# NVlabs/CenterPose

Measured on NVIDIA H100. Metric: images/sec at 512x512 DLA-34 (dla_34 + DCNv2, 7 heads, decode + PnP), higher is better.
Workload: dtype tf32x3

## Files before the change

centerpose_b200/csrc/conv_tma.cu:

```cuda
#include <cuda.h>

#include "common.cuh"
#include "umma_common.cuh"

namespace cp {
namespace {

constexpr int TM_BM = 128;
constexpr int TM_THREADS = 384;
constexpr int TM_THREADS_X3 = 512;

struct TmaConvParams {
  CUtensorMap amap[4];
  int nsrc;
  int srcC[4];
  int B, H, W, Cin, Cout, CoutPad, BN;
  int k;
  int tile_m;
  int Wt, boxh;
  int tiles_per_image;
  long long total_tiles;
  long long m_tiles;
  uint32_t slab_bytes, slab_stride;
  int SA, SB;
  const float* bias;
  const float* residual;
  int resStride, relu, res_after_relu;
  float* out;
  int outStride, out_nchw;
  int round_tf32;
  int cslab;
  int x3;
  int group;
  const unsigned char* wtiles;
  int ksplit, sps;
  float* part;
  int fuse, tph;
  const float* fuse_w[16];
  const float* fuse_b[16];
  float* fuse_out[16];
  int fuse_cout[16];
  int ipm;
  long long wstride, tstride, tiles_per_model;
};

using namespace umma;

struct TmaCtl {
  unsigned long long a_full[4], a_empty[4], a_split[4];
  unsigned long long b_full[8], b_empty[8];
};
static_assert(sizeof(TmaCtl) <= 512, "control block");

struct TileGeo {
  int n_tile, img, g0, r_lo, model;
  long long pos0;
};
template <bool MULTI>
__device__ __forceinline__ TileGeo decode_tile(const TmaConvParams& p, long long ct, int n_tiles) {
  TileGeo g;
  g.n_tile = (int)(ct % n_tiles);
  const long long m_tile = ct / n_tiles;
  g.img = 0;
  g.g0 = 0;
  g.r_lo = 0;
  g.pos0 = 0;
  g.model = 0;
  if (p.k == 3) {
    g.img = (int)(m_tile / p.tiles_per_image);
    g.g0 = (int)(m_tile - (long long)g.img * p.tiles_per_image) * p.tile_m;
    const int t = g.g0 - 1;
    g.r_lo = (t >= 0) ? t / p.Wt : -((-t + p.Wt - 1) / p.Wt);
    if (MULTI) g.model = g.img / p.ipm;
  } else if (MULTI) {
    g.model = (int)(m_tile / p.tiles_per_model);
    g.pos0 = (long long)g.model * p.ipm * p.H * p.W + (m_tile - g.model * p.tiles_per_model) * p.tile_m;
  } else {
    g.pos0 = m_tile * p.tile_m;
  }
  return g;
}

template <bool MULTI>
__device__ __forceinline__ bool tile_position(const TmaConvParams& p, const TileGeo& g, int i, int* n, int* oy, int* ox, int* m) {
  bool valid;
  if (p.k == 3) {
    const int gg = g.g0 + i;
    *oy = gg / p.Wt;
    const int xp = gg - *oy * p.Wt;
    *ox = xp - 1;
    *n = g.img;
    valid = (*oy < p.H) && (xp >= 1) && (xp <= p.W);
  } else {
    const long long pix = g.pos0 + i;
    valid = pix < (MULTI ? (long long)(g.model + 1) * p.ipm : (long long)p.B) * p.H * p.W;
    const long long pp = valid ? pix : 0;
    *ox = (int)(pp % p.W);
    const long long t = pp / p.W;
    *oy = (int)(t % p.H);
    *n = (int)(t / p.H);
  }
  *m = (int)(((size_t)*n * p.H + *oy) * p.W + *ox);
  return valid;
}

template <bool X3, bool FUSE, int BN, bool MULTI>
__global__ void __launch_bounds__(X3 ? TM_THREADS_X3 : TM_THREADS, 1) conv_tma_kernel(const __grid_constant__ TmaConvParams p) {
  extern __shared__ __align__(1024) unsigned char smem[];
  TmaCtl* ctl = reinterpret_cast<TmaCtl*>(smem);
  if (threadIdx.x == 0) griddep_launch_dependents();
  const uint32_t slabs0 = (smem_u32(smem) + 512u + 1023u) & ~1023u;
  const uint32_t rowb = (uint32_t)p.cslab * 4u;
  const uint32_t btile_bytes = (uint32_t)BN * rowb * (X3 ? 2u : 1u);
  const uint32_t a_stage = p.slab_stride * (X3 ? 2u : 1u);
  const uint32_t btiles0 = slabs0 + (uint32_t)p.SA * a_stage;
  const uint32_t drain0 = btiles0 + (uint32_t)p.SB * btile_bytes;

  const int tid = threadIdx.x, warp = tid >> 5, lane = tid & 31;
  const int n_tiles = p.CoutPad / BN;
  const int taps = p.k * p.k;
  const int KS_SPLIT = p.ksplit;
  const int sps = p.sps;
  const int KB = sps * taps;
  const int KB_all = (p.Cin / p.cslab) * taps;
  const long long total_tiles = p.total_tiles;
  const long long tph = FUSE ? p.tph : 1;
  auto tile_at = [&](long long it) { return ((long long)blockIdx.x + (it / tph) * gridDim.x) * tph + (it % tph); };

  if (tid == 0) {
    for (int s = 0; s < p.SA; ++s) {
      mbar_init(smem_u32(&ctl->a_full[s]), 1);
      mbar_init(smem_u32(&ctl->a_empty[s]), 2);
      mbar_init(smem_u32(&ctl->a_split[s]), 128);
    }
    for (int s = 0; s < p.SB; ++s) {
      mbar_init(smem_u32(&ctl->b_full[s]), 1);
      mbar_init(smem_u32(&ctl->b_empty[s]), 2);
    }
    fence_mbar_init();
  }
  __syncthreads();
  if (warp != 1) griddep_wait();

  if (warp < 4) {
    if (X3) asm volatile("setmaxnreg.dec.sync.aligned.u32 40;");
    if (warp == 0) {
      if (lane == 0) {
        int stage = 0;
        uint32_t phase = 0;
        for (long long it = 0, tile = tile_at(0); tile < total_tiles; tile = tile_at(++it)) {
          const TileGeo g = decode_tile<MULTI>(p, tile / KS_SPLIT, n_tiles);
          const int s_begin = (int)(tile % KS_SPLIT) * sps;
          for (int s = s_begin; s < s_begin + sps; ++s) {
            int src = 0, cb = 0;
            while (src + 1 < p.nsrc && s * p.cslab >= cb + p.srcC[src]) {
              cb += p.srcC[src];
              ++src;
            }
            mbar_wait(smem_u32(&ctl->a_empty[stage]), phase ^ 1u);
            const uint32_t bar = smem_u32(&ctl->a_full[stage]);
            mbar_arrive_expect_tx(bar, p.slab_bytes);
            const uint32_t dst = slabs0 + (uint32_t)stage * a_stage;
            if (p.k == 3)
              tma_load_4d(dst, &p.amap[src], s * p.cslab - cb, -1, g.r_lo - 1, g.img, bar);
            else
              tma_load_2d(dst, &p.amap[src], s * p.cslab - cb, (int)g.pos0, bar);
            if (++stage == p.SA) {
              stage = 0;
              phase ^= 1u;
            }
          }
        }
      }
      __syncwarp();
    } else if (warp == 1) {
      if (lane == 0) {
        int stage = 0;
        uint32_t phase = 0;
        for (long long it = 0, tile = tile_at(0); tile < total_tiles; tile = tile_at(++it)) {
          const unsigned char* wsrc;
          if constexpr (MULTI) {
            const TileGeo g = decode_tile<MULTI>(p, tile / KS_SPLIT, n_tiles);
            wsrc = p.wtiles + (size_t)g.model * p.tstride +
                   ((size_t)g.n_tile * KB_all + (size_t)(tile % KS_SPLIT) * KB) * btile_bytes;
          } else {
            const int n_tile = (int)((tile / KS_SPLIT) % n_tiles);
            wsrc = p.wtiles + ((size_t)n_tile * KB_all + (size_t)(tile % KS_SPLIT) * KB) * btile_bytes;
          }
          for (int kb = 0; kb < KB; ++kb) {
            mbar_wait(smem_u32(&ctl->b_empty[stage]), phase ^ 1u);
            const uint32_t bar = smem_u32(&ctl->b_full[stage]);
            mbar_arrive_expect_tx(bar, btile_bytes);
            bulk_g2s(btiles0 + (uint32_t)stage * btile_bytes, wsrc + (size_t)kb * btile_bytes, btile_bytes, bar);
            if (++stage == p.SB) {
              stage = 0;
              phase ^= 1u;
            }
          }
        }
      }
      __syncwarp();
    }
  } else if (X3 && warp >= 12) {
    asm volatile("setmaxnreg.dec.sync.aligned.u32 48;");
    const int st = tid - 384;
    int stage = 0;
    uint32_t phase = 0;
    const uint32_t nchunk = p.slab_bytes >> 4;
    for (long long it = 0, tile = tile_at(0); tile < total_tiles; tile = tile_at(++it)) {
      for (int s = 0; s < sps; ++s) {
        mbar_wait(smem_u32(&ctl->a_full[stage]), phase);
        const uint32_t hi = slabs0 + (uint32_t)stage * a_stage;
        const uint32_t lo = hi + p.slab_stride;
        for (uint32_t c0 = st; c0 < nchunk; c0 += 128 * 4) {
          float4 v[4];
#pragma unroll
          for (int u = 0; u < 4; ++u)
            if (c0 + u * 128 < nchunk) v[u] = ld_shared_v4f(hi + ((c0 + u * 128) << 4));
#pragma unroll
          for (int u = 0; u < 4; ++u) {
            if (c0 + u * 128 < nchunk) {
              float4 h, l;
              h.x = tf32_round(v[u].x); l.x = tf32_round(v[u].x - h.x);
              h.y = tf32_round(v[u].y); l.y = tf32_round(v[u].y - h.y);
              h.z = tf32_round(v[u].z); l.z = tf32_round(v[u].z - h.z);
              h.w = tf32_round(v[u].w); l.w = tf32_round(v[u].w - h.w);
              st_shared_v4f(hi + ((c0 + u * 128) << 4), h.x, h.y, h.z, h.w);
              st_shared_v4f(lo + ((c0 + u * 128) << 4), l.x, l.y, l.z, l.w);
            }
          }
        }
        fence_proxy_async_smem();
        mbar_arrive(smem_u32(&ctl->a_split[stage]));
        if (++stage == p.SA) {
          stage = 0;
          phase ^= 1u;
        }
      }
    }
  } else {
    if (X3) asm volatile("setmaxnreg.inc.sync.aligned.u32 208;");
    const int c = (warp - 4) >> 2, wt = tid & 127;
    float* dstage = reinterpret_cast<float*>(smem + (drain0 - smem_u32(smem))) + (size_t)c * (DRAIN_STAGE_BYTES / 4);
    const uint32_t bar_a = smem_u32(X3 ? &ctl->a_split[0] : &ctl->a_full[0]);
    const uint32_t bar_a_empty = smem_u32(&ctl->a_empty[0]);
    const uint32_t bar_b_full = smem_u32(&ctl->b_full[0]), bar_b_empty = smem_u32(&ctl->b_empty[0]);
    const uint32_t a_lo_u = p.slab_stride >> 4, b_lo_u = ((uint32_t)BN * rowb) >> 4;
    EpiParams ep;
    ep.bias = p.bias;
    ep.residual = p.residual;
    ep.resStride = p.resStride;
    ep.relu = p.relu;
    ep.res_after_relu = p.res_after_relu;
    ep.round_tf32 = p.round_tf32;
    ep.out = p.out;
    ep.outStride = p.outStride;
    ep.out_nchw = p.out_nchw;
    ep.Cout = p.Cout;
    ep.CoutPad = p.CoutPad;
    ep.H = p.H;
    ep.W = p.W;
    int sa = 0, sb = 0;
    uint32_t pa = 0, pb = 0;
    float acc[BN / 2];
    float sums[X3 ? BN / 2 : 1];
    float acc2[FUSE ? 16 : 1];
#pragma unroll
    for (int j = 0; j < BN / 2; ++j) acc[j] = 0.f;
#pragma unroll
    for (int j = 0; j < (FUSE ? 16 : 1); ++j) acc2[j] = 0.f;
    for (long long it = 0, tile = tile_at(0); tile < total_tiles; tile = tile_at(++it)) {
      const TileGeo g = decode_tile<MULTI>(p, tile / KS_SPLIT, n_tiles);
      const uint32_t row0 = (p.k == 3 ? (uint32_t)(g.g0 - 1 - g.r_lo * p.Wt) : 0u) + (uint32_t)c * 64u;
#pragma unroll
      for (int j = 0; j < (X3 ? BN / 2 : 1); ++j) sums[j] = 0.f;
      const int group = X3 ? p.group : 1;
      const bool overlap = X3 && p.SA > 1;
      int tap = 0;
      auto release_prev = [&]() {
        if (wt == 0) {
          mbar_arrive(bar_b_empty + 8u * (uint32_t)(sb == 0 ? p.SB - 1 : sb - 1));
          if (tap == 0) mbar_arrive(bar_a_empty + 8u * (uint32_t)(sa == 0 ? p.SA - 1 : sa - 1));
        }
      };
      for (int kb0 = 0; kb0 < KB; kb0 += group) {
        const int n_kb = min(group, KB - kb0);
        for (int i = 0; i < n_kb; ++i) {
          if (tap == 0) mbar_wait(bar_a + 8u * (uint32_t)sa, pa);
          const int ky = tap / 3, kx = tap - ky * 3;
          const uint32_t arow = row0 + (p.k == 3 ? (uint32_t)(ky * p.Wt + kx) : 0u);
          mbar_wait(bar_b_full + 8u * (uint32_t)sb, pb);
          const uint64_t da = make_desc(slabs0 + (uint32_t)sa * a_stage + arow * rowb, p.cslab);
          const uint64_t db = make_desc(btiles0 + (uint32_t)sb * btile_bytes, p.cslab);
          const bool fresh = X3 ? i == 0 : kb0 == 0;
          if (p.cslab == 32)
            mma_kblock_issue<BN, X3, false, 4>(acc, da, db, a_lo_u, b_lo_u, fresh);
          else
            mma_kblock_issue<BN, X3, false, 2>(acc, da, db, a_lo_u, b_lo_u, fresh);
          if (overlap && i > 0) {
            wg_wait<1>();
            release_prev();
          }
          if (++sb == p.SB) {
            sb = 0;
            pb ^= 1u;
          }
          if (++tap == taps) {
            tap = 0;
            if (++sa == p.SA) {
              sa = 0;
              pa ^= 1u;
            }
          }
          if (!overlap) {
            wg_wait<0>();
            release_prev();
          }
        }
        wg_wait<0>();
        if (overlap) release_prev();
#pragma unroll
        for (int j = 0; j < (X3 ? BN / 2 : 1); ++j)
          if (X3) sums[j] += acc[X3 ? j : 0];
      }
      if (X3) {
#pragma unroll
        for (int j = 0; j < BN / 2; ++j) acc[j] = 0.f;
      }
      const int r_me = wt >> 1;
      int n, oy, ox, m;
      const bool valid = tile_position<MULTI>(p, g, c * 64 + r_me, &n, &oy, &ox, &m);
      const int col_end = min(p.Cout, (g.n_tile + 1) * BN);
      const int head = FUSE ? g.n_tile / p.tph : 0, part = FUSE ? g.n_tile - head * p.tph : 0;
      const size_t wofs = MULTI ? (size_t)g.model * p.wstride : 0;
      if (MULTI) ep.bias = p.bias + wofs;
      if (FUSE && part == 0) {
#pragma unroll
        for (int j = 0; j < (FUSE ? 16 : 1); ++j) acc2[j] = 0.f;
      }
      auto fn = [&](int r, int cb, float (&v)[16]) {
        if (cb >= BN) return;
        if (!FUSE && KS_SPLIT > 1) {
          const long long mn = tile / KS_SPLIT;
          const int ks = (int)(tile % KS_SPLIT);
          float4* mine = reinterpret_cast<float4*>(p.part) + (((size_t)mn * KS_SPLIT + ks) * (BN >> 2) + (cb >> 2)) * p.tile_m +
                         c * 64 + r;
#pragma unroll
          for (int q = 0; q < 4; ++q) __stcg(mine + (size_t)q * p.tile_m, make_float4(v[4 * q], v[4 * q + 1], v[4 * q + 2], v[4 * q + 3]));
        } else if (FUSE) {
          const float* b1 = p.bias + wofs + (size_t)g.n_tile * BN + cb;
          const float4* w2 = reinterpret_cast<const float4*>(p.fuse_w[head] + wofs) + ((size_t)part * BN + cb) * 4;
#pragma unroll
          for (int q = 0; q < 16; ++q) {
            const float h = fmaxf(v[q] + __ldg(b1 + q), 0.f);
#pragma unroll
            for (int u = 0; u < 4; ++u) {
              const float4 w = __ldg(w2 + q * 4 + u);
              acc2[FUSE ? 4 * u + 0 : 0] = fmaf(h, w.x, acc2[FUSE ? 4 * u + 0 : 0]);
              acc2[FUSE ? 4 * u + 1 : 0] = fmaf(h, w.y, acc2[FUSE ? 4 * u + 1 : 0]);
              acc2[FUSE ? 4 * u + 2 : 0] = fmaf(h, w.z, acc2[FUSE ? 4 * u + 2 : 0]);
              acc2[FUSE ? 4 * u + 3 : 0] = fmaf(h, w.w, acc2[FUSE ? 4 * u + 3 : 0]);
            }
          }
        } else {
          epilogue_row<16>(ep, v, valid, m, n, oy, ox, g.n_tile * BN + cb, col_end);
        }
      };
      if constexpr (X3 && FUSE) {
        const int rg = wt >> 3, hh = (wt >> 2) & 1, og = wt & 3;
        const int fr0 = (wt >> 5) * 16 + ((wt & 31) >> 2), fcq = (wt & 3) * 2;
        const float* b1 = p.bias + wofs + (size_t)g.n_tile * BN;
        const float4* w2 = reinterpret_cast<const float4*>(p.fuse_w[head] + wofs) + (size_t)part * BN * 4 + og;
        auto at = [&](int r, int col) { return r * 32 + ((((col >> 2) ^ r) & 7) << 2) + (col & 3); };
#pragma unroll
        for (int c0 = 0; c0 < BN; c0 += 32) {
#pragma unroll
          for (int j = 0; j < BN / 8; ++j) {
            if (j * 8 >= c0 && j * 8 < c0 + 32) {
              const int col = j * 8 - c0 + fcq;
              const float bx = __ldg(b1 + c0 + col), by = __ldg(b1 + c0 + col + 1);
              dstage[at(fr0, col)] = fmaxf(sums[X3 ? 4 * j : 0] + bx, 0.f);
              dstage[at(fr0, col + 1)] = fmaxf(sums[X3 ? 4 * j + 1 : 0] + by, 0.f);
              dstage[at(fr0 + 8, col)] = fmaxf(sums[X3 ? 4 * j + 2 : 0] + bx, 0.f);
              dstage[at(fr0 + 8, col + 1)] = fmaxf(sums[X3 ? 4 * j + 3 : 0] + by, 0.f);
            }
          }
          wg_bar_sync(1 + c);
#pragma unroll
          for (int m4 = 0; m4 < 4; ++m4) {
            const int k0 = 16 * hh + 4 * m4;
            float4 hv[4];
#pragma unroll
            for (int i = 0; i < 4; ++i) hv[i] = *reinterpret_cast<const float4*>(dstage + at(rg + 16 * i, k0));
#pragma unroll
            for (int kk = 0; kk < 4; ++kk) {
              const float4 w = __ldg(w2 + (size_t)(c0 + k0 + kk) * 4);
#pragma unroll
              for (int i = 0; i < 4; ++i) {
                const float h = kk == 0 ? hv[i].x : kk == 1 ? hv[i].y : kk == 2 ? hv[i].z : hv[i].w;
                acc2[FUSE ? 4 * i + 0 : 0] = fmaf(h, w.x, acc2[FUSE ? 4 * i + 0 : 0]);
                acc2[FUSE ? 4 * i + 1 : 0] = fmaf(h, w.y, acc2[FUSE ? 4 * i + 1 : 0]);
                acc2[FUSE ? 4 * i + 2 : 0] = fmaf(h, w.z, acc2[FUSE ? 4 * i + 2 : 0]);
                acc2[FUSE ? 4 * i + 3 : 0] = fmaf(h, w.w, acc2[FUSE ? 4 * i + 3 : 0]);
              }
            }
          }
          wg_bar_sync(1 + c);
        }
        if (part == p.tph - 1) {
#pragma unroll
          for (int j = 0; j < 16; ++j) acc2[FUSE ? j : 0] += __shfl_xor_sync(0xffffffffu, acc2[FUSE ? j : 0], 4);
          if (hh == 0) {
            const int co = p.fuse_cout[head];
            const size_t plane = (size_t)p.H * p.W;
#pragma unroll
            for (int i = 0; i < 4; ++i) {
              int n1, oy1, ox1, m1;
              if (!tile_position<MULTI>(p, g, c * 64 + rg + 16 * i, &n1, &oy1, &ox1, &m1)) continue;
              float* o = p.fuse_out[head] + ((size_t)n1 * co * p.H + oy1) * p.W + ox1;
#pragma unroll
              for (int u = 0; u < 4; ++u)
                if (4 * og + u < co) o[(4 * og + u) * plane] = acc2[FUSE ? 4 * i + u : 0] + __ldg(p.fuse_b[head] + wofs + 4 * og + u);
            }
          }
        }
        continue;
      }
      if constexpr (X3)
        drain_rows<BN>(sums, dstage, wt, 1 + c, fn);
      else
        drain_rows<BN>(acc, dstage, wt, 1 + c, fn);
      if (FUSE && part == p.tph - 1) {
#pragma unroll
        for (int j = 0; j < (FUSE ? 16 : 1); ++j) acc2[j] += __shfl_xor_sync(0xffffffffu, acc2[j], 1);
        if ((wt & 1) == 0 && valid) {
          const int co = p.fuse_cout[head];
          float* o = p.fuse_out[head] + ((size_t)n * co * p.H + oy) * p.W + ox;
          const size_t plane = (size_t)p.H * p.W;
#pragma unroll
          for (int j = 0; j < 16; ++j)
            if (j < co) o[j * plane] = acc2[FUSE ? j : 0] + __ldg(p.fuse_b[head] + wofs + j);
        }
      }
    }
  }
}

__global__ void pack_tma_weight_kernel(const float* __restrict__ src, int ld, int Cin, int taps, int Cout, int BN, int n_tiles,
                                       int round_tf32, int x3, int cslab, unsigned char* __restrict__ dst) {
  const int KB = (Cin / cslab) * taps;
  const int cpr = cslab / 4;
  const size_t rowb = (size_t)cslab * 4;
  const size_t total = (size_t)n_tiles * KB * BN * cpr;
  for (size_t i = blockIdx.x * (size_t)blockDim.x + threadIdx.x; i < total; i += (size_t)gridDim.x * blockDim.x) {
    const int q = i % cpr;
    size_t t = i / cpr;
    const int nr = t % BN;
    t /= BN;
    const int kb = t % KB;
    const int nt = t / KB;
    const int n = nt * BN + nr;
    const int slab = kb / taps, tap = kb - slab * taps;
    float v[4];
#pragma unroll
    for (int j = 0; j < 4; ++j) {
      const int k = tap * Cin + slab * cslab + q * 4 + j;
      float x = (n < Cout) ? src[(size_t)k * ld + n] : 0.f;
      v[j] = round_tf32 ? tf32_round(x) : x;
    }
    const size_t tile = ((size_t)nt * KB + kb) * (size_t)BN * rowb * (x3 ? 2 : 1);
    const int sw = cslab == 32 ? (nr & 7) : ((nr >> 1) & 3);
    const size_t off = (size_t)nr * rowb + (size_t)((q ^ sw) << 4);
    *reinterpret_cast<float4*>(dst + tile + off) = make_float4(v[0], v[1], v[2], v[3]);
    if (x3) {
      float l[4];
#pragma unroll
      for (int j = 0; j < 4; ++j) {
        const int k = tap * Cin + slab * cslab + q * 4 + j;
        const float x = (n < Cout) ? src[(size_t)k * ld + n] : 0.f;
        l[j] = tf32_round(x - v[j]);
      }
      *reinterpret_cast<float4*>(dst + tile + (size_t)BN * rowb + off) = make_float4(l[0], l[1], l[2], l[3]);
    }
  }
}

typedef CUresult (*EncodeTiledFn)(CUtensorMap*, CUtensorMapDataType, cuuint32_t, void*, const cuuint64_t*, const cuuint64_t*,
                                  const cuuint32_t*, const cuuint32_t*, CUtensorMapInterleave, CUtensorMapSwizzle,
                                  CUtensorMapL2promotion, CUtensorMapFloatOOBfill);

EncodeTiledFn get_encode() {
  static EncodeTiledFn fn = nullptr;
  if (!fn) {
    void* p = nullptr;
    cudaDriverEntryPointQueryResult q;
    if (cudaGetDriverEntryPoint("cuTensorMapEncodeTiled", &p, cudaEnableDefault, &q) == cudaSuccess &&
        q == cudaDriverEntryPointSuccess)
      fn = (EncodeTiledFn)p;
  }
  return fn;
}

}

template <bool MULTI>
__global__ void __launch_bounds__(256) conv_tma_splitk_finish(const __grid_constant__ TmaConvParams p, long long mn_tiles) {
  splitk_finish<MULTI>(p, p.tile_m, mn_tiles, [&](long long mn, int i, int* n, int* oy, int* ox) {
    int m;
    return tile_position<MULTI>(p, decode_tile<MULTI>(p, mn, p.CoutPad / p.BN), i, n, oy, ox, &m);
  });
}

static int tma_boxh(int Wt) { return (TM_BM + 1 + 2 * Wt + Wt - 1) / Wt + 1; }

constexpr size_t TM_BUDGET = 222 * 1024 - 2 * (size_t)DRAIN_STAGE_BYTES;

static int tma_smem_layout(uint32_t a_stage, uint32_t btile, int k, int* SA, int* SB, size_t* smem) {
  const size_t budget = TM_BUDGET;
  int sa = 2;
  if ((size_t)sa * a_stage + 2 * (size_t)btile > budget) sa = 1;
  if ((size_t)sa * a_stage + 2 * (size_t)btile > budget) return fail(CP_ERR_INVALID, "conv_tma: slab does not fit shared memory");
  int sb = (int)((budget - (size_t)sa * a_stage) / btile);
  if (sb > 8) sb = 8;
  if (sb < 2) return fail(CP_ERR_INVALID, "conv_tma: tile does not fit shared memory");
  if (k == 1 && sa < 4) {
    int s4 = (int)((budget - (size_t)sb * btile) / a_stage);
    if (s4 > 4) s4 = 4;
    if (s4 > sa) sa = s4;
  }
  *SA = sa;
  *SB = sb;
  *smem = 512 + 2048 + (size_t)sa * a_stage + (size_t)sb * btile + 2 * (size_t)DRAIN_STAGE_BYTES;
  return CP_OK;
}

int tma_cslab(const IgemmParams& p, int x3) {
  if (p.Cin % 32) return 16;
  if (!x3 || p.kh != 3) return 32;
  const int Wt = p.Win + 2;
  const int boxh = tma_boxh(Wt);
  const size_t slab32 = ((size_t)boxh * Wt * 128 + 1023) / 1024 * 1024;
  const int bn = tma_tile_n(p.CoutPad, x3);
  const size_t need = 2 * (2 * slab32) + 2 * ((size_t)bn * 128 * 2);
  return need > TM_BUDGET ? 16 : 32;
}

int tma_tile_n(int CoutPad, int) { return wgmma_tile_n(CoutPad, 128); }

bool tma_conv_supported(const IgemmParams& p, int x3) {
  if (p.mode != IGEMM_NHWC_VEC) return false;
  if (!((p.kh == 1 && p.kw == 1 && p.pad == 0) || (p.kh == 3 && p.kw == 3 && p.pad == 1))) return false;
  if (p.stride != 1) return false;
  const int cs = tma_cslab(p, x3);
  if (p.Cin % cs) return false;
  for (int s = 0; s < p.nsrc; ++s)
    if (p.srcC[s] % cs || p.srcStride[s] % 4) return false;
  if (p.kh == 3 && p.Win + 2 > 256) return false;
  const int bn = tma_tile_n(p.CoutPad, x3);
  if (bn == 0) return false;
  const size_t slab = p.kh == 3 ? (size_t)tma_boxh(p.Win + 2) * (p.Win + 2) * cs * 4 : (size_t)TM_BM * cs * 4;
  const size_t a_stage = ((slab + 1023) / 1024 * 1024) * (x3 ? 2 : 1);
  const size_t btile = (size_t)bn * cs * 4 * (x3 ? 2 : 1);
  return a_stage + 2 * btile <= TM_BUDGET;
}

size_t tma_weight_bytes(int Cin, int taps, int CoutPad, int x3) {
  return (size_t)CoutPad * Cin * taps * 4 * (x3 ? 2 : 1);
}

int launch_pack_tma_weight(const float* src, int ld, int Cin, int taps, int Cout, int CoutPad, int x3, int cs, int bn,
                           void* dst, cudaStream_t s) {
  const int nt = CoutPad / bn;
  size_t total = (size_t)nt * (Cin / cs) * taps * bn * (cs / 4);
  int blocks = (int)((total + 255) / 256);
  if (blocks > 132 * 32) blocks = 132 * 32;
  pack_tma_weight_kernel<<<blocks, 256, 0, s>>>(src, ld, Cin, taps, Cout, bn, nt, 1, x3, cs, (unsigned char*)dst);
  CP_LAUNCH_CHECK("pack_tma_weight_kernel");
  return CP_OK;
}

int tma_encode_nhwc_box(const float* base, int C, int W, int H, int B, int strideFloats, int boxC, int boxW, int boxH,
                        int swizzle64, void* map_out) {
  EncodeTiledFn enc = get_encode();
  if (!enc) return fail(CP_ERR_CUDA, "cuTensorMapEncodeTiled entry point not available");
  cuuint64_t dims[4] = {(cuuint64_t)C, (cuuint64_t)W, (cuuint64_t)H, (cuuint64_t)B};
  cuuint64_t strides[3] = {(cuuint64_t)strideFloats * 4, (cuuint64_t)W * strideFloats * 4, (cuuint64_t)H * W * strideFloats * 4};
  cuuint32_t box[4] = {(cuuint32_t)boxC, (cuuint32_t)boxW, (cuuint32_t)boxH, 1};
  cuuint32_t es[4] = {1, 1, 1, 1};
  CUresult r = enc(reinterpret_cast<CUtensorMap*>(map_out), CU_TENSOR_MAP_DATA_TYPE_FLOAT32, 4, (void*)base, dims, strides, box,
                   es, CU_TENSOR_MAP_INTERLEAVE_NONE, swizzle64 ? CU_TENSOR_MAP_SWIZZLE_64B : CU_TENSOR_MAP_SWIZZLE_NONE,
                   CU_TENSOR_MAP_L2_PROMOTION_L2_256B,
                   CU_TENSOR_MAP_FLOAT_OOB_FILL_NONE);
  if (r != CUDA_SUCCESS) return fail(CP_ERR_CUDA, "cuTensorMapEncodeTiled failed with code " + std::to_string((int)r));
  return CP_OK;
}

int tma_conv_encode(const IgemmParams& p, int Bmax, int cs, void* maps_out) {
  EncodeTiledFn enc = get_encode();
  if (!enc) return fail(CP_ERR_CUDA, "cuTensorMapEncodeTiled entry point not available");
  CUtensorMap* maps = reinterpret_cast<CUtensorMap*>(maps_out);
  const int Wt = p.Win + 2;
  const int boxh = tma_boxh(Wt);
  const CUtensorMapSwizzle swz = cs == 32 ? CU_TENSOR_MAP_SWIZZLE_128B : CU_TENSOR_MAP_SWIZZLE_64B;
  for (int s = 0; s < p.nsrc; ++s) {
    CUresult r;
    if (p.kh == 3) {
      cuuint64_t dims[4] = {(cuuint64_t)p.srcC[s], (cuuint64_t)p.Win, (cuuint64_t)p.Hin, (cuuint64_t)Bmax};
      cuuint64_t strides[3] = {(cuuint64_t)p.srcStride[s] * 4, (cuuint64_t)p.Win * p.srcStride[s] * 4,
                               (cuuint64_t)p.Hin * p.Win * p.srcStride[s] * 4};
      cuuint32_t box[4] = {(cuuint32_t)cs, (cuuint32_t)Wt, (cuuint32_t)boxh, 1};
      cuuint32_t es[4] = {1, 1, 1, 1};
      r = enc(&maps[s], CU_TENSOR_MAP_DATA_TYPE_FLOAT32, 4, (void*)p.src[s], dims, strides, box, es,
              CU_TENSOR_MAP_INTERLEAVE_NONE, swz, CU_TENSOR_MAP_L2_PROMOTION_L2_256B,
              CU_TENSOR_MAP_FLOAT_OOB_FILL_NONE);
    } else {
      cuuint64_t dims[2] = {(cuuint64_t)p.srcC[s], (cuuint64_t)Bmax * p.Hin * p.Win};
      cuuint64_t strides[1] = {(cuuint64_t)p.srcStride[s] * 4};
      cuuint32_t box[2] = {(cuuint32_t)cs, (cuuint32_t)TM_BM};
      cuuint32_t es[2] = {1, 1};
      r = enc(&maps[s], CU_TENSOR_MAP_DATA_TYPE_FLOAT32, 2, (void*)p.src[s], dims, strides, box, es,
              CU_TENSOR_MAP_INTERLEAVE_NONE, swz, CU_TENSOR_MAP_L2_PROMOTION_L2_256B,
              CU_TENSOR_MAP_FLOAT_OOB_FILL_NONE);
    }
    if (r != CUDA_SUCCESS) return fail(CP_ERR_CUDA, "cuTensorMapEncodeTiled failed with code " + std::to_string((int)r));
  }
  return CP_OK;
}

template <bool X3, bool FUSE, bool MULTI>
static int launch_conv_tma_kernel(const TmaConvParams& q, const cudaLaunchConfig_t& cfg0) {
  void (*kern)(TmaConvParams) = nullptr;
  switch (q.BN) {
    case 16: kern = conv_tma_kernel<X3, FUSE, 16, MULTI>; break;
    case 32: kern = conv_tma_kernel<X3, FUSE, 32, MULTI>; break;
    case 64: kern = conv_tma_kernel<X3, FUSE, 64, MULTI>; break;
    case 128: kern = conv_tma_kernel<X3, FUSE, 128, MULTI>; break;
    default: return fail(CP_ERR_INVALID, "conv_tma: unsupported N tile");
  }
  static PerDevice<bool, 4> configured;
  const int slot = q.BN == 128 ? 3 : (q.BN == 64 ? 2 : (q.BN == 32 ? 1 : 0));
  if (!configured.here(slot)) {
    CP_CUDA_CHECK(cudaFuncSetAttribute(kern, cudaFuncAttributeMaxDynamicSharedMemorySize, 227 * 1024));
    configured.here(slot) = true;
  }
  cudaLaunchConfig_t cfg = cfg0;
  cudaLaunchAttribute attr[1];
  attr[0].id = cudaLaunchAttributeProgrammaticStreamSerialization;
  attr[0].val.programmaticStreamSerializationAllowed = 1;
  cfg.attrs = attr;
  cfg.numAttrs = g_pdl ? 1 : 0;
  CP_CUDA_CHECK(cudaLaunchKernelEx(&cfg, kern, q));
  CP_LAUNCH_CHECK("conv_tma_kernel");
  return CP_OK;
}

int launch_conv_tma(const IgemmParams& p, const void* maps, const ConvKernel& k, cudaStream_t stream, LaunchInfo* info) {
  if (!p.wgt_umma) return fail(CP_ERR_INVALID, "conv_tma: weight tiles missing");
  if (p.B % model_ipm(p)) return fail(CP_ERR_INVALID, "conv_tma: batch is not a whole number of models");
  const bool x3 = k.x3;
  TmaConvParams q;
  memset(&q, 0, sizeof(q));
  memcpy(q.amap, maps, sizeof(CUtensorMap) * 4);
  q.nsrc = p.nsrc;
  for (int s = 0; s < 4; ++s) q.srcC[s] = p.srcC[s];
  q.B = p.B;
  q.H = p.Hin;
  q.W = p.Win;
  q.Cin = p.Cin;
  q.Cout = p.Cout;
  q.CoutPad = p.CoutPad;
  q.BN = k.BN;
  q.x3 = x3;
  q.cslab = k.cslab;
  q.group = kX3GroupBlocks * (32 / q.cslab);
  q.k = p.kh;
  q.Wt = p.Win + 2;
  q.tile_m = TM_BM;
  q.boxh = tma_boxh(q.Wt);
  q.ipm = model_ipm(p);
  q.wstride = p.wstride;
  q.tstride = p.tstride;
  size_t m_tiles;
  if (q.k == 3) {
    q.tiles_per_image = (p.Hin * q.Wt + q.tile_m - 1) / q.tile_m;
    m_tiles = (size_t)q.tiles_per_image * p.B;
    q.slab_bytes = (uint32_t)q.boxh * q.Wt * (uint32_t)q.cslab * 4u;
  } else {
    q.tiles_per_image = 0;
    q.tiles_per_model = ((long long)q.ipm * p.Hin * p.Win + q.tile_m - 1) / q.tile_m;
    m_tiles = (size_t)q.tiles_per_model * (p.B / q.ipm);
    q.slab_bytes = (uint32_t)q.tile_m * (uint32_t)q.cslab * 4u;
  }
  q.slab_stride = (q.slab_bytes + 1023u) & ~1023u;
  const uint32_t btile = (uint32_t)q.BN * (uint32_t)q.cslab * 4u * (x3 ? 2u : 1u);
  const uint32_t a_stage = q.slab_stride * (x3 ? 2u : 1u);
  size_t smem = 0;
  if (int rc = tma_smem_layout(a_stage, btile, q.k, &q.SA, &q.SB, &smem)) return rc;
  q.bias = p.bias;
  q.residual = p.residual;
  q.resStride = p.resStride;
  q.relu = p.relu;
  q.res_after_relu = p.res_after_relu;
  q.out = p.out;
  q.outStride = p.outStride;
  q.out_nchw = p.out_nchw;
  q.round_tf32 = k.round_out;
  q.wtiles = (const unsigned char*)p.wgt_umma;
  if (p.fuse_n > 0) {
    if (p.fuse_hidden % q.BN || p.CoutPad != p.fuse_n * p.fuse_hidden || !p.relu || p.residual || (x3 && q.BN != 128))
      return fail(CP_ERR_INVALID, "conv_tma: fused 1x1 needs relu, no residual and head_conv a multiple of the N tile");
    q.fuse = 1;
    q.tph = p.fuse_hidden / q.BN;
    for (int h = 0; h < p.fuse_n; ++h) {
      q.fuse_w[h] = p.fuse_w[h];
      q.fuse_b[h] = p.fuse_b[h];
      q.fuse_out[h] = p.fuse_out[h];
      q.fuse_cout[h] = p.fuse_cout[h];
    }
  }
  q.m_tiles = (long long)m_tiles;
  q.part = p.splitk_ws;
  const long long mn = (long long)m_tiles * (p.CoutPad / q.BN);
  const int nslab = q.Cin / q.cslab;
  int num_sms = 0;
  if (int rc = device_sm_count(&num_sms)) return rc;
  q.ksplit = x3 && !q.fuse ? splitk_factor(mn, nslab, num_sms, (size_t)q.tile_m * q.BN, p.splitk_ws_floats) : 1;
  q.sps = nslab / q.ksplit;
  q.total_tiles = mn * q.ksplit;
  if (q.total_tiles >= (1ll << 31)) return fail(CP_ERR_INVALID, "conv_tma: too many tiles");
  cudaLaunchConfig_t cfg{};
  cfg.gridDim = dim3((unsigned)(q.total_tiles < num_sms ? q.total_tiles : num_sms));
  cfg.blockDim = dim3(x3 ? TM_THREADS_X3 : TM_THREADS);
  cfg.dynamicSmemBytes = smem;
  cfg.stream = stream;
  const bool multi = p.B > q.ipm;
  int rc;
  if (multi)
    rc = x3 ? (q.fuse ? launch_conv_tma_kernel<true, true, true>(q, cfg) : launch_conv_tma_kernel<true, false, true>(q, cfg))
            : (q.fuse ? launch_conv_tma_kernel<false, true, true>(q, cfg) : launch_conv_tma_kernel<false, false, true>(q, cfg));
  else
    rc = x3 ? (q.fuse ? launch_conv_tma_kernel<true, true, false>(q, cfg) : launch_conv_tma_kernel<true, false, false>(q, cfg))
            : (q.fuse ? launch_conv_tma_kernel<false, true, false>(q, cfg) : launch_conv_tma_kernel<false, false, false>(q, cfg));
  if (rc) return rc;
  if (info) {
    info->BN = q.BN;
    info->ksplit = q.ksplit;
    info->grid = cfg.gridDim.x;
  }
  if (q.ksplit > 1) {
    const long long threads = mn * (q.BN / 4) * q.tile_m;
    CP_CUDA_CHECK(launch_kernel(multi ? conv_tma_splitk_finish<true> : conv_tma_splitk_finish<false>,
                                dim3((unsigned)((threads + 255) / 256)), dim3(256), 0, stream, q, mn));
    CP_LAUNCH_CHECK("conv_tma_splitk_finish");
  }
  return CP_OK;
}

}
```

Measured before the change: 740.3.

## Offload fused head 1x1 epilogue to dedicated warpgroup via smem ring

For the tf32x3 fused-head path, adds a fifth warpgroup that runs the second 1x1 conv of each head. The consumer warpgroups now write bias+ReLU hidden activations into a double-buffered shared-memory ring guarded by mbarriers and move on to the next tile, while the new warpgroup stages the 1x1 weights in shared memory and accumulates the outputs. This aims to overlap the scalar FMA epilogue with the tensor-core main loop instead of stalling the MMA warps. In exchange, registers are redistributed across warpgroups (consumers drop to 152), and the ring and weight buffers reduce the shared memory left for pipeline stages.

```diff
diff --git a/centerpose_b200/csrc/conv_tma.cu b/centerpose_b200/csrc/conv_tma.cu
--- a/centerpose_b200/csrc/conv_tma.cu
+++ b/centerpose_b200/csrc/conv_tma.cu
@@ -9,6 +9,9 @@
 constexpr int TM_BM = 128;
 constexpr int TM_THREADS = 384;
 constexpr int TM_THREADS_X3 = 512;
+constexpr int TM_THREADS_X3F = 640;
+constexpr uint32_t TM_HSLOT_BYTES = 128u * 32u * 4u;
+constexpr uint32_t TM_W1_BYTES = 128u * 16u * 4u;
 
 struct TmaConvParams {
   CUtensorMap amap[4];
@@ -42,6 +45,7 @@
   int fuse_cout[16];
   int ipm;
   long long wstride, tstride, tiles_per_model;
+  int RS;
 };
 
 using namespace umma;
@@ -49,6 +53,7 @@
 struct TmaCtl {
   unsigned long long a_full[4], a_empty[4], a_split[4];
   unsigned long long b_full[8], b_empty[8];
+  unsigned long long h_full[2], h_empty[2];
 };
 static_assert(sizeof(TmaCtl) <= 512, "control block");
 
@@ -105,7 +110,10 @@
 }
 
 template <bool X3, bool FUSE, int BN, bool MULTI>
-__global__ void __launch_bounds__(X3 ? TM_THREADS_X3 : TM_THREADS, 1) conv_tma_kernel(const __grid_constant__ TmaConvParams p) {
+__global__ void __launch_bounds__(X3 ? (FUSE ? TM_THREADS_X3F : TM_THREADS_X3) : TM_THREADS, 1)
+    conv_tma_kernel(const __grid_constant__ TmaConvParams p) {
+  constexpr bool EPI = X3 && FUSE;
+  constexpr int REG_CTL = EPI ? 32 : 40, REG_SPLIT = EPI ? 40 : 48, REG_EPI = 104, REG_CONS = EPI ? 152 : 208;
   extern __shared__ __align__(1024) unsigned char smem[];
   TmaCtl* ctl = reinterpret_cast<TmaCtl*>(smem);
   if (threadIdx.x == 0) griddep_launch_dependents();
@@ -137,13 +145,19 @@
       mbar_init(smem_u32(&ctl->b_full[s]), 1);
       mbar_init(smem_u32(&ctl->b_empty[s]), 2);
     }
+    if constexpr (EPI) {
+      for (int s = 0; s < p.RS; ++s) {
+        mbar_init(smem_u32(&ctl->h_full[s]), 256);
+        mbar_init(smem_u32(&ctl->h_empty[s]), 128);
+      }
+    }
     fence_mbar_init();
   }
   __syncthreads();
   if (warp != 1) griddep_wait();
 
   if (warp < 4) {
-    if (X3) asm volatile("setmaxnreg.dec.sync.aligned.u32 40;");
+    if (X3) asm volatile("setmaxnreg.dec.sync.aligned.u32 %0;" ::"n"(REG_CTL));
     if (warp == 0) {
       if (lane == 0) {
         int stage = 0;
@@ -201,8 +215,95 @@
       }
       __syncwarp();
     }
+  } else if (EPI && warp >= 16) {
+    asm volatile("setmaxnreg.inc.sync.aligned.u32 %0;" ::"n"(REG_EPI));
+    const int wt = tid - 512, rg = wt >> 2, hh = (wt >> 1) & 1, og = wt & 1;
+    const float* hring = reinterpret_cast<const float*>(smem + (drain0 - smem_u32(smem)));
+    float4* w1 = reinterpret_cast<float4*>(smem + (drain0 - smem_u32(smem)) + (size_t)p.RS * TM_HSLOT_BYTES);
+    const uint32_t bar_h_full = smem_u32(&ctl->h_full[0]), bar_h_empty = smem_u32(&ctl->h_empty[0]);
+    auto at = [&](int r, int col) { return r * 32 + ((((col >> 2) ^ r) & 7) << 2) + (col & 3); };
+    auto stage_w1 = [&](long long tile) {
+      const TileGeo g = decode_tile<MULTI>(p, tile, n_tiles);
+      const int head = g.n_tile / p.tph, part = g.n_tile - head * p.tph;
+      const float4* src = reinterpret_cast<const float4*>(p.fuse_w[head] + (MULTI ? (size_t)g.model * p.wstride : 0)) +
+                          (size_t)part * BN * 4;
+      for (int i = wt; i < BN * 4; i += 128) w1[i ^ (((i >> 2) & 16) ? 4 : 0)] = __ldg(src + i);
+    };
+    int rs = 0;
+    uint32_t rp = 0;
+    float acc2[32];
+    long long it = 0, tile = tile_at(0);
+    if (tile < total_tiles) stage_w1(tile);
+    wg_bar_sync(3);
+    while (tile < total_tiles) {
+      const TileGeo g = decode_tile<MULTI>(p, tile, n_tiles);
+      const int head = g.n_tile / p.tph, part = g.n_tile - head * p.tph;
+      if (part == 0) {
+#pragma unroll
+        for (int j = 0; j < 32; ++j) acc2[j] = 0.f;
+      }
+#pragma unroll 1
+      for (int c0 = 0; c0 < BN; c0 += 32) {
+        mbar_wait(bar_h_full + 8u * (uint32_t)rs, rp);
+        const float* hs = hring + (size_t)rs * (TM_HSLOT_BYTES / 4);
+#pragma unroll
+        for (int m4 = 0; m4 < 4; ++m4) {
+          const int k0 = 16 * hh + 4 * m4;
+          float4 hv[4];
+#pragma unroll
+          for (int i = 0; i < 4; ++i) hv[i] = *reinterpret_cast<const float4*>(hs + at(rg + 32 * i, k0));
+#pragma unroll
+          for (int kk = 0; kk < 4; ++kk) {
+            const int wi = (((c0 + k0 + kk) << 2) + 2 * og) ^ (hh << 2);
+            const float4 wa = w1[wi], wb = w1[wi + 1];
+#pragma unroll
+            for (int i = 0; i < 4; ++i) {
+              const float h = kk == 0 ? hv[i].x : kk == 1 ? hv[i].y : kk == 2 ? hv[i].z : hv[i].w;
+              acc2[8 * i + 0] = fmaf(h, wa.x, acc2[8 * i + 0]);
+              acc2[8 * i + 1] = fmaf(h, wa.y, acc2[8 * i + 1]);
+              acc2[8 * i + 2] = fmaf(h, wa.z, acc2[8 * i + 2]);
+              acc2[8 * i + 3] = fmaf(h, wa.w, acc2[8 * i + 3]);
+              acc2[8 * i + 4] = fmaf(h, wb.x, acc2[8 * i + 4]);
+              acc2[8 * i + 5] = fmaf(h, wb.y, acc2[8 * i + 5]);
+              acc2[8 * i + 6] = fmaf(h, wb.z, acc2[8 * i + 6]);
+              acc2[8 * i + 7] = fmaf(h, wb.w, acc2[8 * i + 7]);
+            }
+          }
+        }
+        mbar_arrive(bar_h_empty + 8u * (uint32_t)rs);
+        if (++rs == p.RS) {
+          rs = 0;
+          rp ^= 1u;
+        }
+      }
+      if (part == p.tph - 1) {
+#pragma unroll
+        for (int j = 0; j < 32; ++j) acc2[j] += __shfl_xor_sync(0xffffffffu, acc2[j], 2);
+        if (hh == 0) {
+          const int co = p.fuse_cout[head] - 8 * og;
+          const float* b2 = p.fuse_b[head] + (MULTI ? (size_t)g.model * p.wstride : 0) + 8 * og;
+          float bo[8];
+#pragma unroll
+          for (int u = 0; u < 8; ++u) bo[u] = u < co ? __ldg(b2 + u) : 0.f;
+          const size_t plane = (size_t)p.H * p.W;
+#pragma unroll
+          for (int i = 0; i < 4; ++i) {
+            int n1, oy1, ox1, m1;
+            if (!tile_position<MULTI>(p, g, rg + 32 * i, &n1, &oy1, &ox1, &m1)) continue;
+            float* o = p.fuse_out[head] + ((size_t)n1 * p.fuse_cout[head] * p.H + oy1) * p.W + ox1 + 8 * og * plane;
+#pragma unroll
+            for (int u = 0; u < 8; ++u)
+              if (u < co) o[u * plane] = acc2[8 * i + u] + bo[u];
+          }
+        }
+      }
+      tile = tile_at(++it);
+      wg_bar_sync(3);
+      if (tile < total_tiles) stage_w1(tile);
+      wg_bar_sync(3);
+    }
   } else if (X3 && warp >= 12) {
-    asm volatile("setmaxnreg.dec.sync.aligned.u32 48;");
+    asm volatile("setmaxnreg.dec.sync.aligned.u32 %0;" ::"n"(REG_SPLIT));
     const int st = tid - 384;
     int stage = 0;
     uint32_t phase = 0;
@@ -239,7 +340,7 @@
       }
     }
   } else {
-    if (X3) asm volatile("setmaxnreg.inc.sync.aligned.u32 208;");
+    if (X3) asm volatile("setmaxnreg.inc.sync.aligned.u32 %0;" ::"n"(REG_CONS));
     const int c = (warp - 4) >> 2, wt = tid & 127;
     float* dstage = reinterpret_cast<float*>(smem + (drain0 - smem_u32(smem))) + (size_t)c * (DRAIN_STAGE_BYTES / 4);
     const uint32_t bar_a = smem_u32(X3 ? &ctl->a_split[0] : &ctl->a_full[0]);
@@ -327,6 +428,33 @@
 #pragma unroll
         for (int j = 0; j < BN / 2; ++j) acc[j] = 0.f;
       }
+      if constexpr (EPI) {
+        const int fr0 = (wt >> 5) * 16 + ((wt & 31) >> 2), fcq = (wt & 3) * 2;
+        const float* b1 = p.bias + (MULTI ? (size_t)g.model * p.wstride : 0) + (size_t)g.n_tile * BN;
+        float* hring = reinterpret_cast<float*>(smem + (drain0 - smem_u32(smem)));
+        const uint32_t bar_h_full = smem_u32(&ctl->h_full[0]), bar_h_empty = smem_u32(&ctl->h_empty[0]);
+        auto at = [&](int r, int col) { return r * 32 + ((((col >> 2) ^ r) & 7) << 2) + (col & 3); };
+#pragma unroll
+        for (int c0 = 0; c0 < BN; c0 += 32) {
+          const uint32_t chunk = (uint32_t)it * (BN / 32) + c0 / 32;
+          const uint32_t rs = chunk % p.RS, rp = (chunk / p.RS) & 1u;
+          mbar_wait(bar_h_empty + 8u * rs, rp ^ 1u);
+          float* hs = hring + (size_t)rs * (TM_HSLOT_BYTES / 4) + c * 64 * 32;
+#pragma unroll
+          for (int j = 0; j < BN / 8; ++j) {
+            if (j * 8 >= c0 && j * 8 < c0 + 32) {
+              const int col = j * 8 - c0 + fcq;
+              const float bx = __ldg(b1 + c0 + col), by = __ldg(b1 + c0 + col + 1);
+              hs[at(fr0, col)] = fmaxf(sums[X3 ? 4 * j : 0] + bx, 0.f);
+              hs[at(fr0, col + 1)] = fmaxf(sums[X3 ? 4 * j + 1 : 0] + by, 0.f);
+              hs[at(fr0 + 8, col)] = fmaxf(sums[X3 ? 4 * j + 2 : 0] + bx, 0.f);
+              hs[at(fr0 + 8, col + 1)] = fmaxf(sums[X3 ? 4 * j + 3 : 0] + by, 0.f);
+            }
+          }
+          mbar_arrive(bar_h_full + 8u * rs);
+        }
+        continue;
+      }
       const int r_me = wt >> 1;
       int n, oy, ox, m;
       const bool valid = tile_position<MULTI>(p, g, c * 64 + r_me, &n, &oy, &ox, &m);
@@ -366,66 +494,6 @@
           epilogue_row<16>(ep, v, valid, m, n, oy, ox, g.n_tile * BN + cb, col_end);
         }
       };
-      if constexpr (X3 && FUSE) {
-        const int rg = wt >> 3, hh = (wt >> 2) & 1, og = wt & 3;
-        const int fr0 = (wt >> 5) * 16 + ((wt & 31) >> 2), fcq = (wt & 3) * 2;
-        const float* b1 = p.bias + wofs + (size_t)g.n_tile * BN;
-        const float4* w2 = reinterpret_cast<const float4*>(p.fuse_w[head] + wofs) + (size_t)part * BN * 4 + og;
-        auto at = [&](int r, int col) { return r * 32 + ((((col >> 2) ^ r) & 7) << 2) + (col & 3); };
-#pragma unroll
-        for (int c0 = 0; c0 < BN; c0 += 32) {
-#pragma unroll
-          for (int j = 0; j < BN / 8; ++j) {
-            if (j * 8 >= c0 && j * 8 < c0 + 32) {
-              const int col = j * 8 - c0 + fcq;
-              const float bx = __ldg(b1 + c0 + col), by = __ldg(b1 + c0 + col + 1);
-              dstage[at(fr0, col)] = fmaxf(sums[X3 ? 4 * j : 0] + bx, 0.f);
-              dstage[at(fr0, col + 1)] = fmaxf(sums[X3 ? 4 * j + 1 : 0] + by, 0.f);
-              dstage[at(fr0 + 8, col)] = fmaxf(sums[X3 ? 4 * j + 2 : 0] + bx, 0.f);
-              dstage[at(fr0 + 8, col + 1)] = fmaxf(sums[X3 ? 4 * j + 3 : 0] + by, 0.f);
-            }
-          }
-          wg_bar_sync(1 + c);
-#pragma unroll
-          for (int m4 = 0; m4 < 4; ++m4) {
-            const int k0 = 16 * hh + 4 * m4;
-            float4 hv[4];
-#pragma unroll
-            for (int i = 0; i < 4; ++i) hv[i] = *reinterpret_cast<const float4*>(dstage + at(rg + 16 * i, k0));
-#pragma unroll
-            for (int kk = 0; kk < 4; ++kk) {
-              const float4 w = __ldg(w2 + (size_t)(c0 + k0 + kk) * 4);
-#pragma unroll
-              for (int i = 0; i < 4; ++i) {
-                const float h = kk == 0 ? hv[i].x : kk == 1 ? hv[i].y : kk == 2 ? hv[i].z : hv[i].w;
-                acc2[FUSE ? 4 * i + 0 : 0] = fmaf(h, w.x, acc2[FUSE ? 4 * i + 0 : 0]);
-                acc2[FUSE ? 4 * i + 1 : 0] = fmaf(h, w.y, acc2[FUSE ? 4 * i + 1 : 0]);
-                acc2[FUSE ? 4 * i + 2 : 0] = fmaf(h, w.z, acc2[FUSE ? 4 * i + 2 : 0]);
-                acc2[FUSE ? 4 * i + 3 : 0] = fmaf(h, w.w, acc2[FUSE ? 4 * i + 3 : 0]);
-              }
-            }
-          }
-          wg_bar_sync(1 + c);
-        }
-        if (part == p.tph - 1) {
-#pragma unroll
-          for (int j = 0; j < 16; ++j) acc2[FUSE ? j : 0] += __shfl_xor_sync(0xffffffffu, acc2[FUSE ? j : 0], 4);
-          if (hh == 0) {
-            const int co = p.fuse_cout[head];
-            const size_t plane = (size_t)p.H * p.W;
-#pragma unroll
-            for (int i = 0; i < 4; ++i) {
-              int n1, oy1, ox1, m1;
-              if (!tile_position<MULTI>(p, g, c * 64 + rg + 16 * i, &n1, &oy1, &ox1, &m1)) continue;
-              float* o = p.fuse_out[head] + ((size_t)n1 * co * p.H + oy1) * p.W + ox1;
-#pragma unroll
-              for (int u = 0; u < 4; ++u)
-                if (4 * og + u < co) o[(4 * og + u) * plane] = acc2[FUSE ? 4 * i + u : 0] + __ldg(p.fuse_b[head] + wofs + 4 * og + u);
-            }
-          }
-        }
-        continue;
-      }
       if constexpr (X3)
         drain_rows<BN>(sums, dstage, wt, 1 + c, fn);
       else
@@ -514,9 +582,16 @@
 static int tma_boxh(int Wt) { return (TM_BM + 1 + 2 * Wt + Wt - 1) / Wt + 1; }
 
 constexpr size_t TM_BUDGET = 222 * 1024 - 2 * (size_t)DRAIN_STAGE_BYTES;
-
-static int tma_smem_layout(uint32_t a_stage, uint32_t btile, int k, int* SA, int* SB, size_t* smem) {
-  const size_t budget = TM_BUDGET;
+static size_t tma_epi_bytes(int rs) { return (size_t)rs * TM_HSLOT_BYTES + TM_W1_BYTES; }
+
+static int tma_smem_layout(uint32_t a_stage, uint32_t btile, int k, bool epi, int* SA, int* SB, int* RS, size_t* smem) {
+  size_t fixed = 2 * (size_t)DRAIN_STAGE_BYTES;
+  *RS = 0;
+  if (epi) {
+    *RS = 2 * (size_t)a_stage + 3 * (size_t)btile <= 222 * 1024 - tma_epi_bytes(2) ? 2 : 1;
+    fixed = tma_epi_bytes(*RS);
+  }
+  const size_t budget = 222 * 1024 - fixed;
   int sa = 2;
   if ((size_t)sa * a_stage + 2 * (size_t)btile > budget) sa = 1;
   if ((size_t)sa * a_stage + 2 * (size_t)btile > budget) return fail(CP_ERR_INVALID, "conv_tma: slab does not fit shared memory");
@@ -530,7 +605,7 @@
   }
   *SA = sa;
   *SB = sb;
-  *smem = 512 + 2048 + (size_t)sa * a_stage + (size_t)sb * btile + 2 * (size_t)DRAIN_STAGE_BYTES;
+  *smem = 512 + 2048 + (size_t)sa * a_stage + (size_t)sb * btile + fixed;
   return CP_OK;
 }
 
@@ -695,7 +770,7 @@
   const uint32_t btile = (uint32_t)q.BN * (uint32_t)q.cslab * 4u * (x3 ? 2u : 1u);
   const uint32_t a_stage = q.slab_stride * (x3 ? 2u : 1u);
   size_t smem = 0;
-  if (int rc = tma_smem_layout(a_stage, btile, q.k, &q.SA, &q.SB, &smem)) return rc;
+  if (int rc = tma_smem_layout(a_stage, btile, q.k, x3 && p.fuse_n > 0, &q.SA, &q.SB, &q.RS, &smem)) return rc;
   q.bias = p.bias;
   q.residual = p.residual;
   q.resStride = p.resStride;
@@ -730,7 +805,7 @@
   if (q.total_tiles >= (1ll << 31)) return fail(CP_ERR_INVALID, "conv_tma: too many tiles");
   cudaLaunchConfig_t cfg{};
   cfg.gridDim = dim3((unsigned)(q.total_tiles < num_sms ? q.total_tiles : num_sms));
-  cfg.blockDim = dim3(x3 ? TM_THREADS_X3 : TM_THREADS);
+  cfg.blockDim = dim3(x3 ? (q.fuse ? TM_THREADS_X3F : TM_THREADS_X3) : TM_THREADS);
   cfg.dynamicSmemBytes = smem;
   cfg.stream = stream;
   const bool multi = p.B > q.ipm;
```

After: 766.4 (median of 6 runs). 3.5% higher.
